# ashispati/InpaintNet

Hardware: AMD Instinct MI355X
Metric: measures/sec training (MeasureVAE: fwd + CE/KL + bwd + Adam) (higher is better)
Workload: dtype f32; 1 GPU; MeasureVAE training, synthetic FolkDB-shaped tokens, 256 measures per GPU (BASELINE.json configs[1]); V=48,E=10,H=512,Z=256, dropout 0.5, teacher-forcing coin per step, Adam lr=1e-4, every step from the seeded weights; batch_per_gpu=256, global_batch=256, parallelism=dp1

## Files before the change

### inpaintnet_amd/csrc/decode_chain.h

```cpp
#pragma once
#include "chain.h"
#include "sample.h"

constexpr int kDecodeMaxGroups = 8;
constexpr int kDecodeCounterStride = 64;
constexpr int kDecodeStatusWord = kDecodeMaxGroups * kDecodeCounterStride;
constexpr int kDecodeSyncWords = kDecodeStatusWord + 4;

struct DecodeB1Beat {
    const float* z;
    const float* zb_w; const float* zb_b;
    const float* gvec0;
    const float* W_hh0; const float* b_hh0;
    const float* W_ih1; const float* b_ih1; const float* W_hh1; const float* b_hh1;
    const float* bh_w; const float* bh_b;
    const float* bi_w; const float* bi_b;
    const float* wih0_c; long wih0_ld;
};

struct DecodeChainArgs {
    int B, H, T, G, V, members;
    const float* W_hh0; const float* b_hh0;
    const float* cgi;
    const float* table;
    const float* W_ih1; const float* b_ih1; const float* W_hh1; const float* b_hh1;
    const float* W_out; const float* b_out;
    const float* ht0;
    const float* ht0pk;
    float* hx0; float* hx1;
    float* amax;
    unsigned long long* b1ex;
    DecodeB1Beat beat;
    unsigned long long* b1stamps;
    float* weights; long long* samples;
    unsigned* counters; chain::Status status;
    int prezeroed;
    int Bs;
    const float* mask;
    float* hx0m;
    float* sv0; float* sv1; long sv_stride;
    float* h0out;
    float* h1seq;
    sample::Request draw;
};

bool decode_chain_ok(int B, int H, int V, int T, int G);
int launch_decode_chain(DecodeChainArgs a, hipStream_t s);
constexpr int kDecodeB1WordsPerRow = 2 * 35392;
constexpr int kDecodeB1StampWords = 2 * 2 * 32 * 8;
constexpr int kDecodeB1MaxRows = 16;
constexpr int kDecodeB1BeatRowsMax = 6;
constexpr int kDecodeB1OneRowTeamsMax = 3;
int decode_b1_rows(int B);
inline long decode_b1_words(int B) { return (long)decode_b1_rows(B) * kDecodeB1WordsPerRow; }
bool decode_b1_shape_ok(int B, int H, int V, int T, int G, int sample = 0);
bool decode_b1_fused(int Z, int B, int V, int sample = 0);
bool decode_b1_ok(const DecodeChainArgs& a);
int launch_decode_b1(const DecodeChainArgs& a, hipStream_t s);
void decode_b1_set_mode(int m);
int decode_b1_plan_check(int B, int V, int Z, int* out8, int sample = 0);
```

### inpaintnet_amd/csrc/decode_chain.hip

```cpp
#include <cstdio>
#include <cstdlib>
#include "chain.h"
#include "ksplit.h"
#include "prof.h"
#include "decode_chain.h"

using namespace ksplit;

namespace {

template <int MS, int NG, int SQ, class GetB>
__device__ __forceinline__ void contract_b(f32x4 (&acc)[MS][4], const int (&slot)[NG], GetB&& getB,
                                           __amdgpu_buffer_rsrc_t r, int base, int rb0, int rb_last, int S, int s0, int lane) {
    constexpr int CH = SQ < 4 ? SQ : 4, NCH = SQ / CH;
    f32x4 A[2][MS][CH];
    int vo[MS];
    const int oz = chain::opaque_zero();
#pragma unroll
    for (int ms = 0; ms < MS; ++ms) vo[ms] = (((min(rb0 + ms, rb_last) + oz) * S + s0) * 256 + lane * 4) * 4;
    auto load = [&](int c, int buf) {
#pragma unroll
        for (int ms = 0; ms < MS; ++ms)
#pragma unroll
            for (int i = 0; i < CH; ++i) A[buf][ms][i] = chain::ld16_sc1(r, vo[ms] + (c * CH + i) * 1024, base);
    };
    load(0, 0);
    __builtin_amdgcn_sched_barrier(0);
#pragma unroll
    for (int c = 0; c < NCH; ++c) {
        if (c + 1 < NCH) load(c + 1, (c + 1) & 1);
        __builtin_amdgcn_sched_barrier(0);
#pragma unroll
        for (int i = 0; i < CH; ++i) {
            f32x4 Bf[NG];
#pragma unroll
            for (int g = 0; g < NG; ++g) Bf[g] = getB(g, c * CH + i);
#pragma unroll
            for (int e = 0; e < 4; ++e)
#pragma unroll
                for (int ms = 0; ms < MS; ++ms)
#pragma unroll
                    for (int g = 0; g < NG; ++g)
                        acc[ms][slot[g]] = __builtin_amdgcn_mfma_f32_16x16x4f32(A[c & 1][ms][i][e], Bf[g][e], acc[ms][slot[g]], 0, 0, 0);
        }
    }
}

template <int NG, int SQ, int VR, class GetB>
__device__ __forceinline__ void contract_valu(f32x4 (&acc)[1][4], const int (&slot)[NG], GetB&& getB, __amdgpu_buffer_rsrc_t r,
                                              int base, int rb0, int S, int s0, int lane) {
    const int vo = ((rb0 * S + s0) * 256 + lane * 4) * 4;
    f32x4 A[SQ];
#pragma unroll
    for (int si = 0; si < SQ; ++si) A[si] = chain::ld16_sc1(r, vo + si * 1024, base);
    float p[VR][NG];
#pragma unroll
    for (int rr = 0; rr < VR; ++rr)
#pragma unroll
        for (int g = 0; g < NG; ++g) p[rr][g] = 0.f;
    const int src0 = lane & 48;
#pragma unroll
    for (int si = 0; si < SQ; ++si) {
        f32x4 Bf[NG];
#pragma unroll
        for (int g = 0; g < NG; ++g) Bf[g] = getB(g, si);
#pragma unroll
        for (int rr = 0; rr < VR; ++rr) {
#pragma unroll
            for (int e = 0; e < 4; ++e) {
                const float a = __shfl(A[si][e], src0 | rr, 64);
#pragma unroll
                for (int g = 0; g < NG; ++g) p[rr][g] = fmaf(a, Bf[g][e], p[rr][g]);
            }
        }
    }
    const bool q0 = lane < 16;
#pragma unroll
    for (int rr = 0; rr < VR; ++rr)
#pragma unroll
        for (int g = 0; g < NG; ++g) {
            float v = p[rr][g];
            v += __shfl_xor(v, 16, 64);
            v += __shfl_xor(v, 32, 64);
            acc[0][slot[g]][rr] += q0 ? v : 0.f;
        }
}

template <int MS, int NACC>
__device__ __forceinline__ void reduce_tile(const f32x4 (&acc)[MS][4], float* red, int t, float (&out)[MS][NACC]) {
    if constexpr (MS <= 2) {
        reduce_waves<MS, NACC>(acc, red, t, out);
    } else {
        static_assert(MS == 4, "row blocks per group: 1, 2 or 4");
#pragma unroll
        for (int h = 0; h < 2; ++h) {
            f32x4 a2[2][4];
            float o2[2][NACC];
#pragma unroll
            for (int ms = 0; ms < 2; ++ms)
#pragma unroll
                for (int a = 0; a < 4; ++a) a2[ms][a] = acc[2 * h + ms][a];
            if (h) __syncthreads();
            reduce_waves<2, NACC>(a2, red, t, o2);
#pragma unroll
            for (int ms = 0; ms < 2; ++ms)
#pragma unroll
                for (int a = 0; a < NACC; ++a) out[2 * h + ms][a] = o2[ms][a];
        }
    }
}

template <int MS, int SQ, bool TRAIN, int NV = 0, int VR = 0>
__global__ __launch_bounds__(256) void decode_chain_kernel(DecodeChainArgs P) {
    static_assert(NV == 0 || (MS == 1 && !TRAIN && NV <= 4), "redundant logits: small-batch inference only");
    static_assert(VR == 0 || (NV > 0 && VR <= 4), "VALU contraction: the smallest inference batches only");
    constexpr int S = 4 * SQ, H = 64 * SQ;
    extern __shared__ __attribute__((aligned(16))) float smem[];
    float* const wih = smem;
    float* const red = wih + 3 * S * 256;
    float* const xt = red + 4 * 4 * (MS < 2 ? MS : 2) * 256;
    float* const xm = xt + MS * 256;
    unsigned* const flag = reinterpret_cast<unsigned*>(xm + MS * 256);
    int group, member;
    chain::decode_block(blockIdx.x, P.members, group, member);
    const int row0 = group * 16 * MS, B = P.B, T = P.T, V = P.V;
    const int Bs = P.Bs ? P.Bs : B;
    if (row0 >= B) return;
    __builtin_amdgcn_s_setprio(3);
    const int t = threadIdx.x, lane = t & 63;
    const int w = __builtin_amdgcn_readfirstlane(t >> 6);
    const int i16 = lane & 15, q = lane >> 4;
    const int j0 = member * 16, jc = j0 + (t & 15);
    const int rb0 = row0 >> 4, rb_last = (B - 1) >> 4;
    const int pkh = ((B + 15) >> 4) * 16 * H;
    const int NCB = (V + 15) >> 4;
    const bool has_tile = member < NCB * MS;
    const int lp = member / NCB, lcb = member % NCB;

    constexpr int NWO = NV > 0 ? NV : 1;
    f32x4 W0[3][SQ], W1[3][SQ], Wo[NWO][SQ];
#pragma unroll
    for (int g = 0; g < 3; ++g)
#pragma unroll
        for (int si = 0; si < SQ; ++si) {
            const long o = (long)(g * H + j0 + i16) * H + 16 * (w * SQ + si) + 4 * q;
            W0[g][si] = ld4u(P.W_hh0 + o);
            W1[g][si] = ld4u(P.W_hh1 + o);
        }
    if constexpr (NV > 0) {
#pragma unroll
        for (int cb = 0; cb < NV; ++cb)
#pragma unroll
            for (int si = 0; si < SQ; ++si)
                Wo[cb][si] = 16 * cb + i16 < V ? ld4u(P.W_out + (long)(16 * cb + i16) * H + 16 * (w * SQ + si) + 4 * q)
                                               : f32x4{0.f, 0.f, 0.f, 0.f};
    } else {
#pragma unroll
        for (int si = 0; si < SQ; ++si)
            Wo[0][si] = has_tile && 16 * lcb + i16 < V ? ld4u(P.W_out + (long)(16 * lcb + i16) * H + 16 * (w * SQ + si) + 4 * q)
                                                       : f32x4{0.f, 0.f, 0.f, 0.f};
    }
    for (int i = t; i < 3 * S * 64; i += 256) {
        const int ln = i & 63, s = (i >> 6) % S, g = i / (64 * S);
        *reinterpret_cast<f32x4*>(wih + (long)i * 4) = ld4u(P.W_ih1 + (long)(g * H + j0 + (ln & 15)) * H + 16 * s + 4 * (ln >> 4));
    }
    float bh0[3], bi1[3], bh1[3];
#pragma unroll
    for (int g = 0; g < 3; ++g) { bh0[g] = P.b_hh0[g * H + jc]; bi1[g] = P.b_ih1[g * H + jc]; bh1[g] = P.b_hh1[g * H + jc]; }
    const bool col_ok = has_tile && 16 * lcb + (t & 15) < V;
    const float bo = col_ok ? P.b_out[16 * lcb + (t & 15)] : 0.f;
    float bov[NWO];
#pragma unroll
    for (int cb = 0; cb < NWO; ++cb) bov[cb] = NV > 0 && 16 * cb + (t & 15) < V ? P.b_out[16 * cb + (t & 15)] : 0.f;
    long own_tok = 0;
    int brow[MS];
#pragma unroll
    for (int p = 0; p < MS; ++p) brow[p] = min(row0 + ((t + 256 * p) >> 4), B - 1);
    const __amdgpu_buffer_rsrc_t r_hx0 = chain::make_rsrc(P.hx0), r_hx1 = chain::make_rsrc(P.hx1),
                                 r_ht0 = chain::make_rsrc(P.ht0pk), r_am = chain::make_rsrc(P.amax);
    const bool masked = TRAIN && P.mask != nullptr;
    const __amdgpu_buffer_rsrc_t r_hxm = chain::make_rsrc(masked ? P.hx0m : P.hx0);
    unsigned* const counter = P.counters + group * kDecodeCounterStride;
    const chain::Status status = P.status;
    const int members = P.members, G = P.G, nb = T / G;
    const int am_slot = NCB * (((B + 15) >> 4) * 16);
    unsigned phase = 0;
    float hp0[MS], hp1[MS];
    __syncthreads();

    auto token_of = [&](int tick, int p) -> long {
        float best = -1.f;
        int bi = 0;
        for (int cb = 0; cb < NCB; ++cb) {
            const chain::u32x2 u2 = __builtin_amdgcn_raw_buffer_load_b64(r_am, (((tick & 1) * am_slot + cb * (am_slot / NCB) + brow[p]) * 8), 0, 16);
            const unsigned long long u = ((unsigned long long)u2.y << 32) | u2.x;
            const float m = __builtin_bit_cast(float, (unsigned)(u >> 32));
            if (m > best) { best = m; bi = (int)(unsigned)u; }
        }
        return bi;
    };

    for (int tick = 0; tick < T; ++tick) {
        const int beat = tick / G, j = tick % G;
        float c0[MS][3], mk[MS];
#pragma unroll
        for (int p = 0; p < MS; ++p) {
            mk[p] = masked ? P.mask[((long)tick * Bs + brow[p]) * H + jc] : 1.f;
#pragma unroll
            for (int g = 0; g < 3; ++g) c0[p][g] = P.cgi[((long)beat * Bs + brow[p]) * 3 * H + g * H + jc];
            if (j == 0) {
                hp0[p] = P.ht0[((long)beat * Bs + brow[p]) * 2 * H + jc];
                hp1[p] = P.ht0[((long)beat * Bs + brow[p]) * 2 * H + H + jc];
            }
        }
        if (NV == 0 && tick > 0 && !chain::wait_group<chain::K_DECODE_CHAIN>(counter, phase * members, status, &flag[phase & 1])) return;
        long tok[MS];
#pragma unroll
        for (int p = 0; p < MS; ++p) tok[p] = tick == 0 ? V : (NV > 0 ? own_tok : token_of(tick - 1, p));
        if (NV == 0 && tick > 0 && member == 0 && (t & 15) == 0) {
#pragma unroll
            for (int p = 0; p < MS; ++p)
                if (row0 + ((t + 256 * p) >> 4) < B) P.samples[(long)brow[p] * T + tick - 1] = tok[p];
        }
        float g0[MS][3];
#pragma unroll
        for (int p = 0; p < MS; ++p)
#pragma unroll
            for (int g = 0; g < 3; ++g) g0[p][g] = P.table[tok[p] * 3 * H + g * H + jc];
        f32x4 acc[MS][4];
#pragma unroll
        for (int ms = 0; ms < MS; ++ms)
#pragma unroll
            for (int a = 0; a < 4; ++a) acc[ms][a] = f32x4{0.f, 0.f, 0.f, 0.f};
        {
            const int sl[3] = {0, 1, 2};
            auto gb = [&](int g, int si) { return W0[g][si]; };
            if constexpr (VR > 0) {
                if (j == 0) contract_valu<3, SQ, VR>(acc, sl, gb, r_ht0, beat * pkh * 4, rb0, S, w * SQ, lane);
                else contract_valu<3, SQ, VR>(acc, sl, gb, r_hx0, ((tick + 1) & 1) * pkh * 4, rb0, S, w * SQ, lane);
            } else {
                if (j == 0) contract_b<MS, 3, SQ>(acc, sl, gb, r_ht0, beat * pkh * 4, rb0, rb_last, S, w * SQ, lane);
                else contract_b<MS, 3, SQ>(acc, sl, gb, r_hx0, ((tick + 1) & 1) * pkh * 4, rb0, rb_last, S, w * SQ, lane);
            }
        }
        float v[MS][4];
        reduce_tile<MS, 4>(acc, red, t, v);
        float sv[MS][6];
#pragma unroll
        for (int p = 0; p < MS; ++p) {
            const float ghn = v[p][2] + bh0[2];
            const float r = sigmoid_f(v[p][0] + c0[p][0] + g0[p][0] + bh0[0]);
            const float z = sigmoid_f(v[p][1] + c0[p][1] + g0[p][1] + bh0[1]);
            const float n = tanh_f(c0[p][2] + g0[p][2] + r * ghn);
            if (TRAIN) { sv[p][0] = r; sv[p][1] = z; sv[p][2] = n; sv[p][3] = ghn; sv[p][4] = hp0[p]; }
            hp0[p] = (1.f - z) * n + z * hp0[p];
            xt[((t + 256 * p) >> 4) * 16 + (t & 15)] = hp0[p];
            if (TRAIN) {
                sv[p][5] = hp0[p] * mk[p];
                if (masked) xm[((t + 256 * p) >> 4) * 16 + (t & 15)] = sv[p][5];
            }
        }
        __syncthreads();
        if (t < 64 * MS && rb0 + (t >> 6) <= rb_last) {
            chain::publish_block(r_hx0, (tick & 1) * pkh * 4, xt, t >> 6, lane, rb0 + (t >> 6), S, member);
            if (masked) chain::publish_block(r_hxm, beat * pkh * 4, xm, t >> 6, lane, rb0 + (t >> 6), S, member);
        }
        chain::arrive(counter);
        ++phase;
        if (TRAIN) {
#pragma unroll
            for (int p = 0; p < MS; ++p) {
                if (row0 + ((t + 256 * p) >> 4) < B) {
                    const long o = ((long)tick * Bs + brow[p]) * H + jc;
                    if (P.sv0) {
#pragma unroll
                        for (int a = 0; a < 5; ++a) P.sv0[o + a * P.sv_stride] = sv[p][a];
                    }
                    if (P.h0out) P.h0out[o] = sv[p][5];
                }
            }
        }
#pragma unroll
        for (int ms = 0; ms < MS; ++ms)
#pragma unroll
            for (int a = 0; a < 4; ++a) acc[ms][a] = f32x4{0.f, 0.f, 0.f, 0.f};
        {
            const int sh[3] = {0, 1, 3};
            auto gb = [&](int g, int si) { return W1[g][si]; };
            if constexpr (VR > 0) {
                if (j == 0) contract_valu<3, SQ, VR>(acc, sh, gb, r_ht0, (nb + beat) * pkh * 4, rb0, S, w * SQ, lane);
                else contract_valu<3, SQ, VR>(acc, sh, gb, r_hx1, ((tick + 1) & 1) * pkh * 4, rb0, S, w * SQ, lane);
            } else {
                if (j == 0) contract_b<MS, 3, SQ>(acc, sh, gb, r_ht0, (nb + beat) * pkh * 4, rb0, rb_last, S, w * SQ, lane);
                else contract_b<MS, 3, SQ>(acc, sh, gb, r_hx1, ((tick + 1) & 1) * pkh * 4, rb0, rb_last, S, w * SQ, lane);
            }
        }
        if (!chain::wait_group<chain::K_DECODE_CHAIN>(counter, phase * members, status, &flag[phase & 1])) return;
        {
            const int sx[3] = {0, 1, 2};
            auto gb = [&](int g, int si) { return *reinterpret_cast<const f32x4*>(wih + ((g * S + w * SQ + si) * 64 + lane) * 4); };
            if constexpr (VR > 0) contract_valu<3, SQ, VR>(acc, sx, gb, r_hxm, (tick & 1) * pkh * 4, rb0, S, w * SQ, lane);
            else contract_b<MS, 3, SQ>(acc, sx, gb, r_hxm, (masked ? beat : (tick & 1)) * pkh * 4, rb0, rb_last, S, w * SQ, lane);
        }
        reduce_tile<MS, 4>(acc, red, t, v);
#pragma unroll
        for (int p = 0; p < MS; ++p) {
            const float ghn = v[p][3] + bh1[2];
            const float r = sigmoid_f(v[p][0] + bi1[0] + bh1[0]);
            const float z = sigmoid_f(v[p][1] + bi1[1] + bh1[1]);
            const float n = tanh_f(v[p][2] + bi1[2] + r * ghn);
            if (TRAIN) { sv[p][0] = r; sv[p][1] = z; sv[p][2] = n; sv[p][3] = ghn; sv[p][4] = hp1[p]; }
            hp1[p] = (1.f - z) * n + z * hp1[p];
            xt[((t + 256 * p) >> 4) * 16 + (t & 15)] = hp1[p];
        }
        __syncthreads();
        if (t < 64 * MS && rb0 + (t >> 6) <= rb_last)
            chain::publish_block(r_hx1, (tick & 1) * pkh * 4, xt, t >> 6, lane, rb0 + (t >> 6), S, member);
        chain::arrive(counter);
        ++phase;
        if (TRAIN) {
#pragma unroll
            for (int p = 0; p < MS; ++p) {
                if (row0 + ((t + 256 * p) >> 4) < B) {
                    const long o = ((long)tick * Bs + brow[p]) * H + jc;
                    if (P.sv1) {
#pragma unroll
                        for (int a = 0; a < 5; ++a) P.sv1[o + a * P.sv_stride] = sv[p][a];
                    }
                    if (P.h1seq) P.h1seq[o] = hp1[p];
                }
            }
        }
        if (!chain::wait_group<chain::K_DECODE_CHAIN>(counter, phase * members, status, &flag[phase & 1])) return;
        if constexpr (NV > 0) {
            f32x4 la[1][4];
#pragma unroll
            for (int a = 0; a < 4; ++a) la[0][a] = f32x4{0.f, 0.f, 0.f, 0.f};
            int sl[NV];
#pragma unroll
            for (int cb = 0; cb < NV; ++cb) sl[cb] = cb;
            if constexpr (VR > 0) contract_valu<NV, SQ, VR>(la, sl, [&](int g, int si) { return Wo[g][si]; }, r_hx1, (tick & 1) * pkh * 4, rb0,
                                                            S, w * SQ, lane);
            else contract_b<1, NV, SQ>(la, sl, [&](int g, int si) { return Wo[g][si]; }, r_hx1, (tick & 1) * pkh * 4, rb0, rb_last, S,
                                       w * SQ, lane);
            float lv[1][NV];
            reduce_waves<1, NV>(la, red, t, lv);
            const int rl = t >> 4, c = t & 15, b = row0 + rl;
            float m = -1.f;
            int am = 0;
#pragma unroll
            for (int cb = 0; cb < NV; ++cb) {
                const bool okc = 16 * cb + c < V;
                float x = lv[0][cb] + bov[cb];
                x = x > 0.f ? x : 0.f;
                if (member == cb % members && b < B && okc) P.weights[((long)b * T + tick) * V + 16 * cb + c] = x;
                if (!okc) x = -1.f;
                if (x > m) { m = x; am = 16 * cb + c; }
            }
#pragma unroll
            for (int o = 8; o > 0; o >>= 1) {
                const float m2 = __shfl_xor(m, o, 16);
                const int a2 = __shfl_xor(am, o, 16);
                if (m2 > m || (m2 == m && a2 < am)) { m = m2; am = a2; }
            }
            own_tok = am;
            if (member == 0 && c == 0 && b < B) P.samples[(long)b * T + tick] = am;
            continue;
        }
        if (has_tile) {
            f32x4 la[1][4];
            la[0][0] = f32x4{0.f, 0.f, 0.f, 0.f};
            const int s1[1] = {0};
            contract_b<1, 1, SQ>(la, s1, [&](int g, int si) { return Wo[0][si]; }, r_hx1, (tick & 1) * pkh * 4, rb0 + lp, rb_last, S,
                                 w * SQ, lane);
            float lv[1][1];
            reduce_waves<1, 1>(la, red, t, lv);
            const int rl = t >> 4, c = t & 15, b = row0 + 16 * lp + rl;
            float x = lv[0][0] + bo;
            x = x > 0.f ? x : 0.f;
            if (b < B && col_ok) P.weights[((long)b * T + tick) * V + 16 * lcb + c] = x;
            if (!col_ok) x = -1.f;
            float m = x;
            int am = c;
#pragma unroll
            for (int o = 8; o > 0; o >>= 1) {
                const float m2 = __shfl_xor(m, o, 16);
                const int a2 = __shfl_xor(am, o, 16);
                if (m2 > m || (m2 == m && a2 < am)) { m = m2; am = a2; }
            }
            if (c == 0 && rb0 + lp <= rb_last) {
                const unsigned long long u = ((unsigned long long)__builtin_bit_cast(unsigned, m) << 32) | (unsigned)(16 * lcb + am);
                __builtin_amdgcn_raw_buffer_store_b64(chain::u32x2{(unsigned)u, (unsigned)(u >> 32)}, r_am,
                                                      ((tick & 1) * am_slot + lcb * (am_slot / NCB) + row0 + 16 * lp + rl) * 8, 0, 16);
            }
        }
        chain::arrive(counter);
        ++phase;
    }
    if (NV == 0 && member == 0) {
        if (!chain::wait_group<chain::K_DECODE_CHAIN>(counter, phase * members, status, &flag[phase & 1])) return;
        if ((t & 15) == 0) {
#pragma unroll
            for (int p = 0; p < MS; ++p)
                if (row0 + ((t + 256 * p) >> 4) < B) P.samples[(long)brow[p] * T + T - 1] = token_of(T - 1, p);
        }
    }
}

int rows_ms(int B) {
    return (B + 15) / 16 <= kDecodeMaxGroups ? 1 : (B + 31) / 32 <= kDecodeMaxGroups ? 2 : 4;
}
inline int groups_of(int B) { const int ms = rows_ms(B); return (B + 16 * ms - 1) / (16 * ms); }

}

bool decode_chain_ok(int B, int H, int V, int T, int G) {
    if (!chain_enabled() || (H != 256 && H != 512) || B < 1 || V < 1 || V > 128 || T % G != 0) return false;
    if (groups_of(B) > kDecodeMaxGroups || groups_of(B) * (H / 16) > chain_capacity()) return false;
    const int ms = rows_ms(B);
    return ((V + 15) / 16) * ms <= H / 16;
}

size_t decode_chain_lds_bytes(int B, int H) {
    const int ms = rows_ms(B), S = H / 16;
    return (size_t)(3 * S * 256 + 4 * 4 * (ms < 2 ? ms : 2) * 256 + 2 * ms * 256 + 4) * sizeof(float);
}

int launch_decode_chain(DecodeChainArgs a, hipStream_t s) {
    if (!decode_chain_ok(a.B, a.H, a.V, a.T, a.G)) return -1;
    const int ms = rows_ms(a.B), groups = (a.B + 16 * ms - 1) / (16 * ms);
    a.members = a.H / 16;
    if (!a.prezeroed && hipMemsetAsync(a.counters, 0, kDecodeSyncWords * sizeof(unsigned), s) != hipSuccess) return -2;
    a.status = chain_status_for(a.counters + kDecodeStatusWord);
    if (decode_b1_ok(a)) return launch_decode_b1(a, s);
    if (a.beat.z) return -1;
    if (a.draw.uniforms) return -1;
    const size_t lds = decode_chain_lds_bytes(a.B, a.H);
    char label[72];
    const bool train = a.sv0 || a.sv1 || a.mask || a.h0out || a.h1seq;
    if (a.mask && !a.hx0m) return -1;
    std::snprintf(label, sizeof label, "decode_chain%s ms%d T%d B%d H%d V%d", train ? "_train" : (a.B == 1 ? "_valu" : ""), ms, a.T, a.B, a.H, a.V);
    ProfScope prof(PROF_GRU_FWD, 2.0 * a.T * a.B * (9.0 * a.H * a.H + (double)a.V * a.H), s, label,
                   4.0 * (9.0 * a.H * a.H + (double)a.V * a.H + (double)a.B * a.T * a.V +
                          (train ? 13.0 * a.T * a.B * a.H : 0.0)));
    const dim3 grid(chain::blocks_for(groups, a.members));
#define DISPATCH_DC5(M, Q, TR, NVV, VRR)                                                                                    \
    do {                                                                                                                \
        static bool attr = false;                                                                                       \
        if (!attr) {                                                                                                    \
            (void)hipFuncSetAttribute(reinterpret_cast<const void*>(&decode_chain_kernel<M, Q, TR, NVV, VRR>),            \
                                      hipFuncAttributeMaxDynamicSharedMemorySize, 160 * 1024);                          \
            attr = true;                                                                                                \
        }                                                                                                               \
        hipLaunchKernelGGL((decode_chain_kernel<M, Q, TR, NVV, VRR>), grid, dim3(256), lds, s, a);                      \
    } while (0)
#define DISPATCH_DC4(M, Q, TR, NVV) DISPATCH_DC5(M, Q, TR, NVV, 0)
#define DISPATCH_DC(M, Q, TR) DISPATCH_DC4(M, Q, TR, 0)
    if (train) {
        if (a.H == 512) { if (ms == 1) DISPATCH_DC(1, 8, true); else if (ms == 2) DISPATCH_DC(2, 8, true); else DISPATCH_DC(4, 8, true); }
        else { if (ms == 1) DISPATCH_DC(1, 4, true); else if (ms == 2) DISPATCH_DC(2, 4, true); else DISPATCH_DC(4, 4, true); }
    } else {
        const int nv = (ms == 1 && a.V <= 64) ? (a.V <= 48 ? 3 : 4) : 0;
        const int vr = (nv > 0 && a.B == 1) ? 1 : 0;
        if (nv == 3 && vr == 1) { if (a.H == 512) DISPATCH_DC5(1, 8, false, 3, 1); else DISPATCH_DC5(1, 4, false, 3, 1); }
        else if (nv == 4 && vr == 1) { if (a.H == 512) DISPATCH_DC5(1, 8, false, 4, 1); else DISPATCH_DC5(1, 4, false, 4, 1); }
        else if (nv == 3) { if (a.H == 512) DISPATCH_DC4(1, 8, false, 3); else DISPATCH_DC4(1, 4, false, 3); }
        else if (nv == 4) { if (a.H == 512) DISPATCH_DC4(1, 8, false, 4); else DISPATCH_DC4(1, 4, false, 4); }
        else if (a.H == 512) { if (ms == 1) DISPATCH_DC(1, 8, false); else if (ms == 2) DISPATCH_DC(2, 8, false); else DISPATCH_DC(4, 8, false); }
        else { if (ms == 1) DISPATCH_DC(1, 4, false); else if (ms == 2) DISPATCH_DC(2, 4, false); else DISPATCH_DC(4, 4, false); }
    }
#undef DISPATCH_DC
#undef DISPATCH_DC4
#undef DISPATCH_DC5
    return hipGetLastError() == hipSuccess ? 0 : -2;
}
```

### inpaintnet_amd/csrc/vae.hip

```cpp
#include "seq.h"
#include "layout.h"
#include "vae.h"
#include "decode_chain.h"
#include "sample.h"
#include <cstdlib>
#include <string>

namespace {

struct EncWs {
    float *tabF, *tabR, *hcat, *a_mu, *a_ls;
    BiGru2Ws g;
    float *d_amu, *d_als, *dhcat, *onehot, *dtab;
};

size_t enc_carve(const inet_vae_config& c, int B, int save, void* base, EncWs& w) {
    Carver cv(base);
    const int T = c.beats * c.ticks_per_beat, H = c.enc_hidden, V = c.num_notes, E = c.emb_dim;
    w.tabF = cv.take<float>((size_t)V * 3 * H);
    w.tabR = cv.take<float>((size_t)V * 3 * H);
    w.hcat = cv.take<float>((size_t)B * 4 * H);
    w.a_mu = cv.take<float>((size_t)B * 2 * H);
    w.a_ls = cv.take<float>((size_t)B * 2 * H);
    bigru2_carve(cv, B, T, H, save, w.g);
// ... 467 lines not shown
    else { P0.h_prev = w.h0seq + (long)(t - 1) * BH; P0.ld_hprev = H; }
    P0.W_hh = p + L.tick[0].w_hh; P0.b_hh = p + L.tick[0].b_hh;
    P0.gi_dense = w.cgi + (long)i * B * 3 * H; P0.ld_gi = 3L * H;
    P0.gi_table = w.table; P0.ld_table = 3L * H;
    if (t == 0) { P0.idx = w.idxV; P0.idx_stride = 1; }
    else { P0.idx = d.samples + (t - 1); P0.idx_stride = T; }
    P0.h_new = w.h0seq + (long)t * BH; P0.ld_hnew = H;
    if (d.mask_tick) { P0.h_masked = w.h0m + (long)t * BH; P0.ld_hm = H; P0.mask = d.mask_tick + (long)t * BH; P0.ld_mask = H; }
    P1.B = B;
    if (j == 0) { P1.h_prev = w.ht0 + (long)i * B * 2 * H + H; P1.ld_hprev = 2L * H; }
    else { P1.h_prev = w.h1seq + (long)(t - 1) * BH; P1.ld_hprev = H; }
    P1.W_hh = p + L.tick[1].w_hh; P1.b_hh = p + L.tick[1].b_hh;
    P1.x = (d.mask_tick ? w.h0m : w.h0seq) + (long)t * BH; P1.ldx = H; P1.K2 = H;
    P1.W_ih = p + L.tick[1].w_ih; P1.ld_wih = H; P1.b_ih = p + L.tick[1].b_ih;
    P1.h_new = w.h1seq + (long)t * BH; P1.ld_hnew = H;
    const auto saves = [&](GruFwdProb& P, float* q) { P.sv_r = q; P.sv_z = q + as; P.sv_n = q + 2 * as; P.sv_ghn = q + 3 * as; P.sv_hprev = q + 4 * as; };
    if (d.save) { saves(P0, w.svt0 + (long)t * BH); saves(P1, w.svt1 + (long)t * BH); }
    if (d.r.pk) tick_pk(w, i, j, d.nb, d.pkh, d.mask_tick != nullptr, P0, P1);
}

int dec_ticks_tf_steps(const DecCall& d) {
    for (int j = 0; j < d.G; ++j) {
        GruFwdBatch b0{}, b1{};
        b0.H = b1.H = d.H; b0.nprob = b1.nprob = d.nb;
        for (int i = 0; i < d.nb; ++i) dec_tick_probs(d, i, j, b0.p[i], b1.p[i]);
        INET_TRY(launch_gru_fwd(b0, d.s));
        INET_TRY(launch_gru_fwd(b1, d.s));
    }
    return dec_project_tf(d);
}

int dec_ticks_fused(const DecCall& d) {
    const DecWs& w = d.w; const VaeLayout& L = d.L; const float* p = d.p; hipStream_t s = d.s;
    const int B = d.B, nb = d.nb, T = d.T, H = d.H, V = d.V;
    const bool chunked = d.r.ticks == kFusedChunked;
    const int Bc = chunked ? d.r.chunk_rows : B;
    const long pkc = (long)pk_floats(Bc, H);
    for (int r0 = 0; r0 < B; r0 += Bc) {
        if (d.r.ht0 == kHt0PerChunk)
            for (int l = 0; l < 2; ++l)
                INET_TRY(pw_pack_frag(w.ht0 + (long)r0 * 2 * H + (long)l * H, 2L * H, Bc, H, w.ht0pk + (long)l * nb * pkc, 0, nb,
                                      (long)B * 2 * H, pkc, s));
        DecodeChainArgs a{};
        a.B = Bc; a.Bs = B; a.H = H; a.T = T; a.G = d.G; a.V = V;
        a.W_hh0 = p + L.tick[0].w_hh; a.b_hh0 = p + L.tick[0].b_hh;
        a.cgi = w.cgi + (long)r0 * 3 * H; a.table = w.table;
        a.W_ih1 = p + L.tick[1].w_ih; a.b_ih1 = p + L.tick[1].b_ih; a.W_hh1 = p + L.tick[1].w_hh; a.b_hh1 = p + L.tick[1].b_hh;
        a.W_out = p + L.out_w; a.b_out = p + L.out_b;
        a.ht0 = w.ht0 + (long)r0 * 2 * H; a.ht0pk = w.ht0pk;
        a.hx0 = w.hpk_t0; a.hx1 = w.hpk_t1; a.amax = w.amax;
        a.b1ex = d.r.b1 ? reinterpret_cast<unsigned long long*>(w.b1ex) : nullptr;
        static const bool b1st = [] { const char* v = std::getenv("INET_DECODE_B1_STAMPS"); return v && v[0] == '1'; }();
        a.b1stamps = (d.r.b1 && b1st && T <= 32) ? reinterpret_cast<unsigned long long*>(w.b1stamps) : nullptr;
        if (d.r.b1_fused) {
            DecodeB1Beat& bt = a.beat;
            bt.z = d.z; bt.zb_w = p + L.zb_w; bt.zb_b = p + L.zb_b; bt.gvec0 = w.gvec0;
            bt.W_hh0 = p + L.beat[0].w_hh; bt.b_hh0 = p + L.beat[0].b_hh;
            bt.W_ih1 = p + L.beat[1].w_ih; bt.b_ih1 = p + L.beat[1].b_ih; bt.W_hh1 = p + L.beat[1].w_hh; bt.b_hh1 = p + L.beat[1].b_hh;
            bt.bh_w = p + L.bh_w; bt.bh_b = p + L.bh_b; bt.bi_w = p + L.bi_w; bt.bi_b = p + L.bi_b;
            bt.wih0_c = d.wih0 + d.E; bt.wih0_ld = d.ldw0;
        }
        a.weights = d.weights + (long)r0 * T * V; a.samples = d.samples + (long)r0 * T;
        SyncArea sa;
        INET_TRY(d.areas->take(kDecAreaFused, &sa));
        a.counters = sa.counters; a.prezeroed = sa.prezeroed;
        a.draw = d.rq;
        if (d.mask_tick) { a.mask = d.mask_tick + (long)r0 * H; a.hx0m = w.hm0pk; }
        if (d.save) {
            a.sv0 = w.svt0 + (long)r0 * H; a.sv1 = w.svt1 + (long)r0 * H; a.sv_stride = (long)T * d.BH;
            a.h0out = (d.mask_tick ? w.h0m : w.h0seq) + (long)r0 * H; a.h1seq = w.h1seq + (long)r0 * H;
        }
        INET_TRY(launch_decode_chain(a, s));
    }
    return 0;
}

int dec_ticks_per_tick(const DecCall& d) {
    const DecWs& w = d.w; const VaeLayout& L = d.L; const float* p = d.p; hipStream_t s = d.s;
    const int B = d.B, T = d.T, H = d.H, V = d.V;
    const bool draw = d.seed != 0;
    for (int t = 0; t < T; ++t) {
        GruFwdBatch b0{}, b1{};
        b0.H = b1.H = H; b0.nprob = b1.nprob = 1;
        dec_tick_probs(d, t / d.G, t % d.G, b0.p[0], b1.p[0]);
        INET_TRY(launch_gru_fwd(b0, s));
        INET_TRY(launch_gru_fwd(b1, s));
        const float* h1 = w.h1seq + (long)t * d.BH;
        float* wt = d.weights + (long)t * V;
        int rc = draw || d.sampled ? 1 : launch_logits_argmax(h1, H, B, H, p + L.out_w, p + L.out_b, V, wt, (long)T * V, d.samples + t, T, s,
                                                               d.r.pk ? b1.p[0].hpk_new : nullptr, w.wpk_out);
        if (rc < 0) return rc;
        if (rc == 1) {
            INET_TRY(linear_fwd(h1, H, p + L.out_w, H, p + L.out_b, wt, (long)T * V, B, V, H, EPI_RELU, s));
            if (draw) INET_TRY(pw_sample_multinomial(wt, (long)T * V, B, V, d.samples + t, T, d.seed, (uint64_t)t * B, s));
            else if (d.sampled) INET_TRY(pw_sample(wt, (long)T * V, B, V, d.samples + t, T, d.rq.tick(t, V), d.level, s));
            else INET_TRY(pw_argmax(wt, (long)T * V, B, V, d.samples + t, T, s));
        }
    }
    return 0;
}

}

size_t vae_decoder_ws_bytes(const inet_vae_config& c, int B, int save) {
    DecWs w{};
    return dec_carve(c, B, save, nullptr, w);
}

int vae_decoder_fwd(const inet_vae_config& c, int B, const float* z, const long long* target, int teacher_forced,
                    const float* p, const float* mask_beat, const float* mask_tick, float* weights,
                    long long* samples, void* ws, int save, hipStream_t s, uint64_t multinomial_seed, const sample::Request& rq) {
    if (c.beats > 4) return -1;
    if (teacher_forced && !target) return -1;
    const bool sampled = rq.uniforms != nullptr;
    if (sampled && (teacher_forced || multinomial_seed)) return -1;
    if (!rq.ok(c.num_notes) || rq.logits) return -1;
    DecCall d(c);
    d.B = B; d.nb = c.beats; d.G = c.ticks_per_beat; d.T = d.nb * d.G; d.H = c.dec_hidden; d.V = c.num_notes; d.E = c.emb_dim; d.Z = c.z_dim;
    d.BH = (long)B * d.H; d.pkh = (long)pk_floats(B, d.H);
    d.save = save; d.teacher_forced = teacher_forced; d.sampled = sampled;
    d.level = rq.level(d.V);
    d.z = z; d.p = p; d.mask_beat = mask_beat; d.mask_tick = mask_tick; d.target = target; d.weights = weights; d.samples = samples;
    d.wih0 = p + d.L.tick[0].w_ih; d.ldw0 = d.E + d.H;
    d.seed = multinomial_seed; d.rq = rq; d.s = s;
    dec_carve(c, B, save, ws, d.w);
    d.r = dec_route(c, B, save, teacher_forced != 0, multinomial_seed != 0, mask_beat != nullptr, mask_tick != nullptr, d.level, sampled, d.w);
    INET_TRY(dec_prologue(d));
    SyncLedger areas = dec_ledger(d.r, d.w);
    d.areas = &areas;
    INET_TRY(dec_pack_weights(d));
    if (d.r.beats != kBeatsFolded) INET_TRY(dec_beat_path(d));
    switch (d.r.ticks) {
        case kTfChained: return dec_ticks_tf_chained(d);
        case kTfSteps: return dec_ticks_tf_steps(d);
        case kFused: case kFusedChunked: return dec_ticks_fused(d);
        default: return dec_ticks_per_tick(d);
    }
}

int vae_decoder_route(const inet_vae_config& c, int B, int save, int teacher_forced, int flags, int level, int32_t* out, int n_out) {
    const bool sampled = level > 0;
    if (c.beats > 4 || level < 0 || level > 4 || !out || n_out < 13) return -1;
    if (sampled && (teacher_forced || (flags & 1))) return -1;
    DecWs w{};
    dec_carve(c, B, save, reinterpret_cast<char*>(static_cast<uintptr_t>(1) << 30), w);
    const DecRoute r = dec_route(c, B, save, teacher_forced != 0, (flags & 1) != 0, (flags & 2) != 0, (flags & 4) != 0, level, sampled, w);
    const int32_t v[16] = {r.beats, r.ticks, r.npl, r.chunk_rows, r.b1, r.b1_fused, r.zero, r.pack_beat, r.pack_tick, r.pack_out, r.ht0, r.pk,
                           r.fused_prezeroed, (int32_t)r.beat_areas, (int32_t)r.tick_areas, r.self_zeroed};
    for (int i = 0; i < (n_out >= 16 ? 16 : 13); ++i) out[i] = v[i];
    return 0;
}


int vae_decoder_bwd(const inet_vae_config& c, int B, const float* dweights, const float* weights,
                    const long long* tokens_in, const float* p, float* g, const float* mask_beat,
                    const float* mask_tick, float* dz, void* ws, hipStream_t s) {
    const int nb = c.beats, G = c.ticks_per_beat, T = nb * G, H = c.dec_hidden, V = c.num_notes, E = c.emb_dim, Z = c.z_dim;
    const long BH = (long)B * H, TBH = (long)T * BH;
    VaeLayout L(c);
    DecWs w{};
    dec_carve(c, B, 1, ws, w);
    const GruDirOff* gr[4] = {&L.beat[0], &L.beat[1], &L.tick[0], &L.tick[1]};
    const bool beats_chained = w.wpkT[0] && w.dghpk && chain_chunk_rows_bwd(H, B, nb, 1) > 0;
    const bool ticks_chained = w.wpkT[0] && w.dghpk && chain_chunk_rows_bwd(H, B, G, nb) > 0;
    if (hipMemsetAsync(w.sync, 0, (size_t)((char*)(w.tmp3h + 3 * H) - (char*)w.sync), s) != hipSuccess) return -2;
    SyncLedger areas(w.sync);
    areas.zeroed_all();
    if (w.wpkT[0]) {
        const float* ins[4]; float* outs[4];
        int n = 0;
        for (int i = 0; i < 4; ++i)
            if (!(i < 2 ? beats_chained : ticks_chained)) { ins[n] = p + gr[i]->w_hh; outs[n++] = w.wpkT[i]; }
        if (n) INET_TRY(pw_pack_frag_multi(ins, outs, n, H, H, 3 * H, 1, s));
    } else {
        for (int i = 0; i < 4; ++i) INET_TRY(pw_transpose(p + gr[i]->w_hh, H, w.whhT[i], 3L * H, 3 * H, H, s));
    }
    const long pkg = (long)pk_floats(B, 3 * H);

    INET_TRY(pw_dlogits_relayout(dweights, weights, B, T, V, w.dlg, s));
    INET_TRY(linear_dgrad(w.dlg, V, p + L.out_w, H, w.dh1top, H, T * B, V, H, EPI_NONE, nullptr, 0, ACC_STORE, s));

    int dcgi_done = 0;
    const auto tick_dir_bwd = [&](int layer, int i) {
        DirBwd D{};
        D.W_hhT = w.whhT[2 + layer];
        D.dout = (layer ? w.dh1top : w.dx1t) + (long)i * G * BH; D.dout_ld = H; D.dout_ts = BH;
        D.sv = (layer ? w.svt1 : w.svt0) + (long)i * G * BH; D.sv_astride = TBH;
        D.dgi = (layer ? w.dgi1t : w.dgi0t) + (long)i * G * 3 * BH; D.dgi_ld = 3L * H; D.dgi_ts = 3 * BH;
        D.dgh = (layer ? w.dgh1t : w.dgh0t) + (long)i * G * 3 * BH;
        D.dhz = w.dhz + (long)i * 2 * BH;
        if (g) { D.db_ih = g + L.tick[layer].b_ih; D.db_hh = g + L.tick[layer].b_hh; }
        D.dh0 = w.dht0 + (long)i * B * 2 * H + layer * H; D.dh0_ld = 2L * H; D.dh0_acc = 0;
        D.Wpk_hhT = w.wpkT[2 + layer]; D.dghpk = w.dghpk ? w.dghpk + (long)i * 3 * pkg : nullptr;
        if (ticks_chained) { D.W_hh = p + L.tick[layer].w_hh; D.areas = &areas; D.area = dec_area_bwd_tick(layer); }
        if (layer == 0) { D.dgi_sum = w.dcgi + (long)i * 3 * BH; D.dgi_sum_done = &dcgi_done; }
        return D;
    };
    DirBwd d[4];
    for (int i = 0; i < nb; ++i) d[i] = tick_dir_bwd(1, i);
    INET_TRY(gru_layer_bwd(H, B, G, nb, d, s));
    const float* x1 = mask_tick ? w.h0m : w.h0seq;
    INET_TRY(linear_dgrad(w.dgi1t, 3L * H, p + L.tick[1].w_ih, H, w.dx1t, H, T * B, 3 * H, H,
                          mask_tick ? EPI_MUL_AUX : EPI_NONE, mask_tick, H, ACC_STORE, s));

    for (int i = 0; i < nb; ++i) d[i] = tick_dir_bwd(0, i);
    INET_TRY(gru_layer_bwd(H, B, G, nb, d, s));
    const float* wih0 = p + L.tick[0].w_ih;
    const long ldw0 = E + H;
    if (!dcgi_done) INET_TRY(pw_group_sum(w.dgi0t, nb, G, 3 * BH, w.dcgi, s));
    INET_TRY(linear_dgrad(w.dcgi, 3L * H, wih0 + E, ldw0, w.dc_all, H, nb * B, 3 * H, H, EPI_MUL_SELU_GRAD, w.c_all, H,
                          ACC_STORE, s));
    if (g) {
        hipStream_t ss = side_fork(s);
        INET_TRY(linear_wgrad2(w.dgh1t, w.dgi1t, 3L * H, w.svt1 + 4 * TBH, x1, H, g + L.tick[1].w_hh, g + L.tick[1].w_ih, H,
                               T * B, 3 * H, H, ss));
        INET_TRY(linear_wgrad(w.dlg, V, w.h1seq, H, g + L.out_w, H, T * B, V, H, ss));
        INET_TRY(pw_colsum(w.dlg, V, T * B, V, g + L.out_b, ss));
        INET_TRY(gru_dir_wgrad(H, B, T, w.dgh0t, w.svt0 + 4 * TBH, g + L.tick[0].w_hh, ss));
        INET_TRY(linear_wgrad(w.dcgi, 3L * H, w.c_all, H, g + L.tick[0].w_ih + E, ldw0, nb * B, 3 * H, H, ss));
        if (!w.onehot) {
            INET_TRY(pw_shift_tokens(tokens_in, B, T, V, w.tokin, ss));
            INET_TRY(pw_token_segsum(w.dgi0t, 3L * H, w.tokin, B, 1, T, T * B, V + 1, 3 * H, w.dtable, ss));
            const float* wih[1] = {wih0};
            float* dwih[1] = {g + L.tick[0].w_ih};
            INET_TRY(pw_table_grad(w.dtable, V + 1, 3 * H, 1, E, p + L.dec_emb, E, wih, dwih, ldw0, g + L.dec_emb, E, ss,
                                   p + L.x_0, g + L.x_0));
        } else {
        INET_TRY(pw_zero(w.onehot, (long)T * B * (V + 1), ss));
        INET_TRY(pw_onehot(w.idxV, B, 0, 1, B, V + 1, w.onehot, 0, ss));
        INET_TRY(pw_onehot(tokens_in, B, 1, T, (T - 1) * B, V + 1, w.onehot + (long)B * (V + 1), 0, ss));
        INET_TRY(launch_gemm(gemm_args(w.onehot, V + 1, 1, w.dgi0t, 3L * H, 1, w.dtable, 3L * H, V + 1, 3 * H, T * B), ss));
        INET_TRY(linear_wgrad(w.dtable, 3L * H, p + L.dec_emb, E, g + L.tick[0].w_ih, ldw0, V, 3 * H, E, ss));
        INET_TRY(linear_wgrad(w.dtable + (long)V * 3 * H, 3L * H, p + L.x_0, E, g + L.tick[0].w_ih, ldw0, 1, 3 * H, E, ss));
        INET_TRY(linear_dgrad(w.dtable, 3L * H, wih0, ldw0, g + L.dec_emb, E, V, 3 * H, E, EPI_NONE, nullptr, 0, ACC_ADD, ss));
        INET_TRY(linear_dgrad(w.dtable + (long)V * 3 * H, 3L * H, wih0, ldw0, g + L.x_0, E, 1, 3 * H, E, EPI_NONE, nullptr, 0, ACC_ADD, ss));
        }
    }

    INET_TRY(pw_mul(w.dht0, w.ht0, 2L * nb * BH, 1, s));
    INET_TRY(linear_dgrad(w.dht0, 2L * H, p + L.bh_w, H, w.dbeat_out, H, nb * B, 2 * H, H, EPI_NONE, nullptr, 0, ACC_STORE, s));
    INET_TRY(linear_dgrad(w.dc_all, H, p + L.bi_w, H, w.dbeat_out, H, nb * B, H, H, EPI_NONE, nullptr, 0, ACC_ADD, s));

    const auto beat_dir_bwd = [&](int layer) {
        DirBwd b{};
        b.W_hhT = w.whhT[layer];
        b.dout = layer ? w.dbeat_out : w.dxb; b.dout_ld = H; b.dout_ts = BH;
        b.sv = layer ? w.svb1 : w.svb0; b.sv_astride = nb * BH;
        b.dgi = layer ? w.dgi1b : w.dgi0b; b.dgi_ld = 3L * H; b.dgi_ts = 3 * BH;
        b.dgh = layer ? w.dgh1b : w.dgh0b; b.dhz = w.dhz;
        if (g) { b.db_ih = g + L.beat[layer].b_ih; b.db_hh = g + L.beat[layer].b_hh; }
        b.dh0 = w.dhb0 + layer * H; b.dh0_ld = 2L * H;
        b.Wpk_hhT = w.wpkT[layer]; b.dghpk = w.dghpk;
        if (beats_chained) { b.W_hh = p + L.beat[layer].w_hh; b.areas = &areas; b.area = dec_area_bwd_beat(layer); }
        return b;
    };
    DirBwd b = beat_dir_bwd(1);
    INET_TRY(gru_layer_bwd(H, B, nb, 1, &b, s));
    const float* xb = mask_beat ? w.beat0m : w.beat0;
    INET_TRY(linear_dgrad(w.dgi1b, 3L * H, p + L.beat[1].w_ih, H, w.dxb, H, nb * B, 3 * H, H,
                          mask_beat ? EPI_MUL_AUX : EPI_NONE, mask_beat, H, ACC_STORE, s));
    b = beat_dir_bwd(0);
    INET_TRY(gru_layer_bwd(H, B, nb, 1, &b, s));

    INET_TRY(pw_mul(w.dhb0, w.hb0, 2 * BH, 1, s));
    if (dz) INET_TRY(linear_dgrad(w.dhb0, 2L * H, p + L.zb_w, Z, dz, Z, B, 2 * H, Z, EPI_NONE, nullptr, 0, ACC_STORE, s));
    if (g) {
        hipStream_t ss = side_fork(s);
        const GemmArgs ga[4] = {linear_wgrad_args(w.dht0, 2L * H, w.beat_out, H, g + L.bh_w, H, nb * B, 2 * H, H),
                                linear_wgrad_args(w.dc_all, H, w.beat_out, H, g + L.bi_w, H, nb * B, H, H),
                                linear_wgrad_args(w.dgh1b, 3L * H, w.svb1 + 4 * nb * BH, H, g + L.beat[1].w_hh, H, nb * B, 3 * H, H),
                                linear_wgrad_args(w.dgi1b, 3L * H, xb, H, g + L.beat[1].w_ih, H, nb * B, 3 * H, H)};
        INET_TRY(launch_gemm_group(ga, 4, ss));
        const GemmArgs gb[2] = {linear_wgrad_args(w.dgh0b, 3L * H, w.svb0 + 4 * nb * BH, H, g + L.beat[0].w_hh, H, nb * B, 3 * H, H),
                                linear_wgrad_args(w.dhb0, 2L * H, w.zsave, Z, g + L.zb_w, Z, B, 2 * H, Z)};
        INET_TRY(launch_gemm_group(gb, 2, ss));
        const PwColsumJob cs[4] = {{w.dht0, 2L * H, nb * B, 2 * H, g + L.bh_b}, {w.dc_all, H, nb * B, H, g + L.bi_b},
                                   {w.dhb0, 2L * H, B, 2 * H, g + L.zb_b}, {w.dgi0b, 3L * H, nb * B, 3 * H, w.tmp3h}};
        INET_TRY(pw_colsum_multi(cs, 4, ss));
        INET_TRY(pw_beat_input_grad(w.tmp3h, p + L.beat[0].w_ih, 1, p + L.b_0, g + L.beat[0].w_ih, g + L.b_0, 3 * H,
                                    w.dgi0b, 3L * H, nb * B, w.b0part, ss));
    }
    return side_join(s);
}

int vae_ws_field(const inet_vae_config& c, int B, int which, const char* name, long long* offset_floats, long long* count) {
    char* const base = reinterpret_cast<char*>(static_cast<uintptr_t>(1) << 30);
    const long long nb = c.beats;
    const float* p = nullptr;
    long long n = 0;
    const std::string f(name ? name : "");
    if (which == 0) {
        EncWs w;
        enc_carve(c, B, 1, base, w);
        const long long H = c.enc_hidden;
        if (f == "a_mu") { p = w.a_mu; n = (long long)B * 2 * H; }
        else if (f == "a_ls") { p = w.a_ls; n = (long long)B * 2 * H; }
    } else if (which == 1) {
        DecWs w{};
        dec_carve(c, B, 1, base, w);
        const long long H = c.dec_hidden;
        if (f == "hb0") { p = w.hb0; n = (long long)B * 2 * H; }
        else if (f == "ht0") { p = w.ht0; n = nb * B * 2 * H; }
        else if (f == "c_all") { p = w.c_all; n = nb * B * H; }
    }
    else if (which == 2) {
        DecWs w{};
        dec_carve(c, B, 0, base, w);
        if (f == "b1stamps" && w.b1stamps) { p = reinterpret_cast<const float*>(w.b1stamps); n = kDecodeB1StampWords; }
    }
    if (!p) return -1;
    if (offset_floats) *offset_floats = (reinterpret_cast<const char*>(p) - base) / (long long)sizeof(float);
    if (count) *count = n;
    return 0;
}
```

Before: 71000 measures/s.

## Hoist next-tick layer-0 recurrent contraction before group wait; cache gather table in LDS

Result: no change. 71340 measures/s, median of 6 (+0.5%).

```diff
diff --git a/inpaintnet_amd/csrc/decode_chain.h b/inpaintnet_amd/csrc/decode_chain.h
--- a/inpaintnet_amd/csrc/decode_chain.h
+++ b/inpaintnet_amd/csrc/decode_chain.h
@@ -1,8 +1,8 @@
 #pragma once
 #include "chain.h"
 #include "sample.h"
+#include "decode_chain_lds.h"
 
-constexpr int kDecodeMaxGroups = 8;
 constexpr int kDecodeCounterStride = 64;
 constexpr int kDecodeStatusWord = kDecodeMaxGroups * kDecodeCounterStride;
 constexpr int kDecodeSyncWords = kDecodeStatusWord + 4;
diff --git a/inpaintnet_amd/csrc/decode_chain.hip b/inpaintnet_amd/csrc/decode_chain.hip
--- a/inpaintnet_amd/csrc/decode_chain.hip
+++ b/inpaintnet_amd/csrc/decode_chain.hip
@@ -43,6 +43,20 @@
                     for (int g = 0; g < NG; ++g)
                         acc[ms][slot[g]] = __builtin_amdgcn_mfma_f32_16x16x4f32(A[c & 1][ms][i][e], Bf[g][e], acc[ms][slot[g]], 0, 0, 0);
         }
+    }
+}
+
+template <int K> using kc = std::integral_constant<int, K>;
+template <int MS, int SQ, int K0, int K1, class GetB>
+__device__ __forceinline__ void contract_ks(f32x4 (&acc)[MS][4], const int (&slot)[3], GetB&& getB, __amdgpu_buffer_rsrc_t r, int base,
+                                            int rb0, int rb_last, int S, int s0, int lane) {
+    if constexpr (K0 == 0 && K1 == SQ) {
+        contract_b<MS, 3, SQ>(acc, slot, getB, r, base, rb0, rb_last, S, s0, lane);
+    } else if constexpr (K1 - K0 > 4) {
+        contract_b<MS, 3, 4>(acc, slot, [&](int g, int si) { return getB(g, K0 + si); }, r, base, rb0, rb_last, S, s0 + K0, lane);
+        contract_ks<MS, SQ, K0 + 4, K1>(acc, slot, getB, r, base, rb0, rb_last, S, s0, lane);
+    } else if constexpr (K1 > K0) {
+        contract_b<MS, 3, K1 - K0>(acc, slot, [&](int g, int si) { return getB(g, K0 + si); }, r, base, rb0, rb_last, S, s0 + K0, lane);
     }
 }
 
@@ -121,6 +135,12 @@
     float* const xt = red + 4 * 4 * (MS < 2 ? MS : 2) * 256;
     float* const xm = xt + MS * 256;
     unsigned* const flag = reinterpret_cast<unsigned*>(xm + MS * 256);
+    float* const tab = xm + MS * 256 + 4;
+    constexpr bool HOIST = VR == 0 && !(MS == 4 && SQ == 8);
+    constexpr int Q = SQ / 4;
+    constexpr int L0A = !HOIST ? 0 : NV > 0 ? 4 : 1;
+    constexpr bool TAB = !(MS == 4 && SQ == 8);
+    static_assert(!TAB || decode_tab_floats(MS, 64 * SQ, 128) > 0, "the gather-table slice must fit at V = 128");
     int group, member;
     chain::decode_block(blockIdx.x, P.members, group, member);
     const int row0 = group * 16 * MS, B = P.B, T = P.T, V = P.V;
@@ -164,6 +184,11 @@
         const int ln = i & 63, s = (i >> 6) % S, g = i / (64 * S);
         *reinterpret_cast<f32x4*>(wih + (long)i * 4) = ld4u(P.W_ih1 + (long)(g * H + j0 + (ln & 15)) * H + 16 * s + 4 * (ln >> 4));
     }
+    const int tabf = TAB ? decode_tab_floats(MS, H, V) : 0;
+    for (int i = t; i < tabf; i += 256) {
+        const int row = i / 48, gc = i - row * 48;
+        tab[i] = P.table[(long)row * 3 * H + (gc >> 4) * H + j0 + (gc & 15)];
+    }
     float bh0[3], bi1[3], bh1[3];
 #pragma unroll
     for (int g = 0; g < 3; ++g) { bh0[g] = P.b_hh0[g * H + jc]; bi1[g] = P.b_ih1[g * H + jc]; bh1[g] = P.b_hh1[g * H + jc]; }
@@ -188,6 +213,26 @@
     float hp0[MS], hp1[MS];
     __syncthreads();
 
+    f32x4 acc0[MS][4];
+    auto zero = [&](f32x4 (&a)[MS][4]) {
+#pragma unroll
+        for (int ms = 0; ms < MS; ++ms)
+#pragma unroll
+            for (int k = 0; k < 4; ++k) a[ms][k] = f32x4{0.f, 0.f, 0.f, 0.f};
+    };
+    auto part0 = [&](f32x4 (&a)[MS][4], auto k0, auto k1, int tn, int bn, int jn) {
+        constexpr int K0 = decltype(k0)::value, K1 = decltype(k1)::value;
+        const int sl[3] = {0, 1, 2};
+        auto gb = [&](int g, int si) { return W0[g][si]; };
+        if constexpr (VR > 0) {
+            static_assert(K0 == 0 && K1 == SQ, "the VALU builds contract the whole k range at once");
+            if (jn == 0) contract_valu<3, SQ, VR>(a, sl, gb, r_ht0, bn * pkh * 4, rb0, S, w * SQ, lane);
+            else contract_valu<3, SQ, VR>(a, sl, gb, r_hx0, ((tn + 1) & 1) * pkh * 4, rb0, S, w * SQ, lane);
+        } else {
+            if (jn == 0) contract_ks<MS, SQ, K0, K1>(a, sl, gb, r_ht0, bn * pkh * 4, rb0, rb_last, S, w * SQ, lane);
+            else contract_ks<MS, SQ, K0, K1>(a, sl, gb, r_hx0, ((tn + 1) & 1) * pkh * 4, rb0, rb_last, S, w * SQ, lane);
+        }
+    };
     auto token_of = [&](int tick, int p) -> long {
         float best = -1.f;
         int bi = 0;
@@ -200,8 +245,13 @@
         return bi;
     };
 
-    for (int tick = 0; tick < T; ++tick) {
-        const int beat = tick / G, j = tick % G;
+    float v0[MS][3];
+    if constexpr (HOIST) {
+        zero(acc0);
+        part0(acc0, kc<0>{}, kc<SQ>{}, 0, 0, 0);
+        reduce_tile<MS, 3>(acc0, red, t, v0);
+    }
+    for (int tick = 0, beat = 0, j = 0; tick < T; ++tick, j = j + 1 == G ? 0 : j + 1, beat += j == 0) {
         float c0[MS][3], mk[MS];
 #pragma unroll
         for (int p = 0; p < MS; ++p) {
@@ -226,31 +276,25 @@
 #pragma unroll
         for (int p = 0; p < MS; ++p)
 #pragma unroll
-            for (int g = 0; g < 3; ++g) g0[p][g] = P.table[tok[p] * 3 * H + g * H + jc];
-        f32x4 acc[MS][4];
-#pragma unroll
-        for (int ms = 0; ms < MS; ++ms)
-#pragma unroll
-            for (int a = 0; a < 4; ++a) acc[ms][a] = f32x4{0.f, 0.f, 0.f, 0.f};
-        {
-            const int sl[3] = {0, 1, 2};
-            auto gb = [&](int g, int si) { return W0[g][si]; };
-            if constexpr (VR > 0) {
-                if (j == 0) contract_valu<3, SQ, VR>(acc, sl, gb, r_ht0, beat * pkh * 4, rb0, S, w * SQ, lane);
-                else contract_valu<3, SQ, VR>(acc, sl, gb, r_hx0, ((tick + 1) & 1) * pkh * 4, rb0, S, w * SQ, lane);
-            } else {
-                if (j == 0) contract_b<MS, 3, SQ>(acc, sl, gb, r_ht0, beat * pkh * 4, rb0, rb_last, S, w * SQ, lane);
-                else contract_b<MS, 3, SQ>(acc, sl, gb, r_hx0, ((tick + 1) & 1) * pkh * 4, rb0, rb_last, S, w * SQ, lane);
-            }
-        }
-        float v[MS][4];
-        reduce_tile<MS, 4>(acc, red, t, v);
+            for (int g = 0; g < 3; ++g)
+                g0[p][g] = TAB ? tab[(int)tok[p] * 48 + g * 16 + (t & 15)] : P.table[tok[p] * 3 * H + g * H + jc];
+        if constexpr (!HOIST) {
+            f32x4 acc[MS][4];
+            zero(acc);
+            part0(acc, kc<0>{}, kc<SQ>{}, tick, beat, j);
+            float v[MS][4];
+            reduce_tile<MS, 4>(acc, red, t, v);
+#pragma unroll
+            for (int p = 0; p < MS; ++p)
+#pragma unroll
+                for (int g = 0; g < 3; ++g) v0[p][g] = v[p][g];
+        }
         float sv[MS][6];
 #pragma unroll
         for (int p = 0; p < MS; ++p) {
-            const float ghn = v[p][2] + bh0[2];
-            const float r = sigmoid_f(v[p][0] + c0[p][0] + g0[p][0] + bh0[0]);
-            const float z = sigmoid_f(v[p][1] + c0[p][1] + g0[p][1] + bh0[1]);
+            const float ghn = v0[p][2] + bh0[2];
+            const float r = sigmoid_f(v0[p][0] + c0[p][0] + g0[p][0] + bh0[0]);
+            const float z = sigmoid_f(v0[p][1] + c0[p][1] + g0[p][1] + bh0[1]);
             const float n = tanh_f(c0[p][2] + g0[p][2] + r * ghn);
             if (TRAIN) { sv[p][0] = r; sv[p][1] = z; sv[p][2] = n; sv[p][3] = ghn; sv[p][4] = hp0[p]; }
             hp0[p] = (1.f - z) * n + z * hp0[p];
@@ -280,10 +324,8 @@
                 }
             }
         }
-#pragma unroll
-        for (int ms = 0; ms < MS; ++ms)
-#pragma unroll
-            for (int a = 0; a < 4; ++a) acc[ms][a] = f32x4{0.f, 0.f, 0.f, 0.f};
+        f32x4 acc[MS][4];
+        zero(acc);
         {
             const int sh[3] = {0, 1, 3};
             auto gb = [&](int g, int si) { return W1[g][si]; };
@@ -302,6 +344,7 @@
             if constexpr (VR > 0) contract_valu<3, SQ, VR>(acc, sx, gb, r_hxm, (tick & 1) * pkh * 4, rb0, S, w * SQ, lane);
             else contract_b<MS, 3, SQ>(acc, sx, gb, r_hxm, (masked ? beat : (tick & 1)) * pkh * 4, rb0, rb_last, S, w * SQ, lane);
         }
+        float v[MS][4];
         reduce_tile<MS, 4>(acc, red, t, v);
 #pragma unroll
         for (int p = 0; p < MS; ++p) {
@@ -330,6 +373,11 @@
                     if (P.h1seq) P.h1seq[o] = hp1[p];
                 }
             }
+        }
+        const int bn = j + 1 == G ? beat + 1 : beat, jn = j + 1 == G ? 0 : j + 1;
+        if (HOIST && tick + 1 < T) {
+            if constexpr (L0A > 0) { zero(acc0); part0(acc0, kc<0>{}, kc<L0A * Q>{}, tick + 1, bn, jn); }
+            if constexpr (L0A == 4) reduce_tile<MS, 3>(acc0, red, t, v0);
         }
         if (!chain::wait_group<chain::K_DECODE_CHAIN>(counter, phase * members, status, &flag[phase & 1])) return;
         if constexpr (NV > 0) {
@@ -396,6 +444,13 @@
         }
         chain::arrive(counter);
         ++phase;
+        if (HOIST && tick + 1 < T) {
+            if constexpr (L0A < 4) {
+                if constexpr (L0A == 0) zero(acc0);
+                part0(acc0, kc<L0A * Q>{}, kc<SQ>{}, tick + 1, bn, jn);
+                reduce_tile<MS, 3>(acc0, red, t, v0);
+            }
+        }
     }
     if (NV == 0 && member == 0) {
         if (!chain::wait_group<chain::K_DECODE_CHAIN>(counter, phase * members, status, &flag[phase & 1])) return;
@@ -407,9 +462,7 @@
     }
 }
 
-int rows_ms(int B) {
-    return (B + 15) / 16 <= kDecodeMaxGroups ? 1 : (B + 31) / 32 <= kDecodeMaxGroups ? 2 : 4;
-}
+inline int rows_ms(int B) { return decode_rows_ms(B); }
 inline int groups_of(int B) { const int ms = rows_ms(B); return (B + 16 * ms - 1) / (16 * ms); }
 
 }
@@ -419,11 +472,6 @@
     if (groups_of(B) > kDecodeMaxGroups || groups_of(B) * (H / 16) > chain_capacity()) return false;
     const int ms = rows_ms(B);
     return ((V + 15) / 16) * ms <= H / 16;
-}
-
-size_t decode_chain_lds_bytes(int B, int H) {
-    const int ms = rows_ms(B), S = H / 16;
-    return (size_t)(3 * S * 256 + 4 * 4 * (ms < 2 ? ms : 2) * 256 + 2 * ms * 256 + 4) * sizeof(float);
 }
 
 int launch_decode_chain(DecodeChainArgs a, hipStream_t s) {
@@ -435,7 +483,8 @@
     if (decode_b1_ok(a)) return launch_decode_b1(a, s);
     if (a.beat.z) return -1;
     if (a.draw.uniforms) return -1;
-    const size_t lds = decode_chain_lds_bytes(a.B, a.H);
+    const size_t lds = decode_chain_lds_bytes(a.B, a.H, a.V);
+    if (lds > (size_t)kDecodeLdsMaxBytes) return -1;
     char label[72];
     const bool train = a.sv0 || a.sv1 || a.mask || a.h0out || a.h1seq;
     if (a.mask && !a.hx0m) return -1;
diff --git a/inpaintnet_amd/csrc/decode_chain_lds.h b/inpaintnet_amd/csrc/decode_chain_lds.h
--- /dev/null
+++ b/inpaintnet_amd/csrc/decode_chain_lds.h
@@ -0,0 +1,15 @@
+#pragma once
+#include <cstddef>
+
+constexpr int kDecodeMaxGroups = 8;
+constexpr int kDecodeLdsMaxBytes = 160 * 1024;
+
+constexpr int decode_rows_ms(int B) { return (B + 15) / 16 <= kDecodeMaxGroups ? 1 : (B + 31) / 32 <= kDecodeMaxGroups ? 2 : 4; }
+constexpr int decode_lds_base_floats(int ms, int H) { return 3 * (H / 16) * 256 + 4 * 4 * (ms < 2 ? ms : 2) * 256 + 2 * ms * 256 + 4; }
+constexpr int decode_tab_floats(int ms, int H, int V) {
+    return (ms == 4 && H == 512) ? 0
+         : (decode_lds_base_floats(ms, H) + (V + 1) * 48) * (int)sizeof(float) <= kDecodeLdsMaxBytes ? (V + 1) * 48 : 0;
+}
+constexpr size_t decode_chain_lds_bytes(int B, int H, int V) {
+    return (size_t)(decode_lds_base_floats(decode_rows_ms(B), H) + decode_tab_floats(decode_rows_ms(B), H, V)) * sizeof(float);
+}
diff --git a/inpaintnet_amd/csrc/vae.hip b/inpaintnet_amd/csrc/vae.hip
--- a/inpaintnet_amd/csrc/vae.hip
+++ b/inpaintnet_amd/csrc/vae.hip
@@ -793,6 +793,12 @@
         if (f == "hb0") { p = w.hb0; n = (long long)B * 2 * H; }
         else if (f == "ht0") { p = w.ht0; n = nb * B * 2 * H; }
         else if (f == "c_all") { p = w.c_all; n = nb * B * H; }
+        const long long TBH = nb * c.ticks_per_beat * B * H;
+        if (f == "svt0") { p = w.svt0; n = 5 * TBH; }
+        else if (f == "svt1") { p = w.svt1; n = 5 * TBH; }
+        else if (f == "h0seq") { p = w.h0seq; n = TBH; }
+        else if (f == "h0m") { p = w.h0m; n = TBH; }
+        else if (f == "h1seq") { p = w.h1seq; n = TBH; }
     }
     else if (which == 2) {
         DecWs w{};
```
